# alibaba/pairec

Hardware: AMD Instinct MI355X
Metric: ranked items/sec, 5k-cand DNN rank (recall top-5000 of 100M x 128 -> DNN3 -> fuse -> sort) (higher is better)
Workload: dtype bf16x3; 1 GPU; configs[1]+[2]: recall 5k of 100000000x128 fp32 table in HBM -> 3-layer DNN rank (256-512-256-1, bf16 MFMA with split hi + lo operands = bf16x3, fp32-accurate scores) -> RankScore fusion (fp64) -> ItemRankScore sort; candidates_per_request=5000, table_rows=100000000, dim=128, table_dist=uniform, batches_in_flight=2, contexts=2, all_batches_on_predicted_thresholds=True, batches_re_run_after_a_failed_plan=0, parallelism=1 GPU

## Files before the change

### pairec_amd/csrc/common.hpp

```cpp
#pragma once
#include <hip/hip_runtime.h>

#include <algorithm>
#include <cstdarg>
#include <cstdint>
#include <cstdio>
#include <cstring>
#include <map>
#include <atomic>
#include <memory>
#include <mutex>
#include <shared_mutex>
#include <string>
#include <vector>

#include "../../include/pairec_gpu.h"

namespace pg {

struct PipeRun;
void set_error(const char* fmt, ...);

#define PG_HIP(expr)                                                                           \
    do {                                                                                       \
// ... 440 lines not shown
int ensure_table_r2(pg_ctx* ctx, const pg_table* tc);
int rescreen16_prep_launch(pg_ctx* ctx, const pg_table* t, const RecallScratch& rs, uint32_t nq);
int rescreen16_launch(pg_ctx* ctx, const pg_table* t, const RecallScratch& rs, uint32_t nq);
int screen4m_launch(pg_ctx* ctx, const pg_table* t, const RecallScratch& rs, uint32_t nq, uint32_t row_begin, uint32_t row_end,
                    uint32_t cap1, bool susp2_clean = false);
int topk_merge_strided_locked(pg_ctx* ctx, const uint64_t* d_rows, const float* d_scores, uint32_t nq, uint32_t nlists,
                              uint32_t per_list, size_t row_ls, size_t row_qs, size_t sc_ls, size_t sc_qs, uint32_t k,
                              uint64_t* d_out_rows, float* d_out_scores, uint32_t* d_out_count);
int topk_merge_locked(pg_ctx* ctx, const uint64_t* d_rows, const float* d_scores, uint32_t nq, uint32_t nlists,
                      uint32_t per_list, int list_major, uint32_t k, uint64_t* d_out_rows, float* d_out_scores,
                      uint32_t* d_out_count);

int rank_dnn3_dev_locked(pg_ctx* ctx, const pg_model* m, const pg_table* t, const float* d_user,
                         const uint32_t* d_cand, const uint32_t* d_off, uint32_t n_req, uint32_t n_items,
                         float* d_out, size_t out_stride = 0);
int fm2t_user_embedding_locked(pg_ctx* ctx, const pg_model* m, const float* d_user, uint32_t n_req, float* d_out);
int rank_fm2t_irows_dev_locked(pg_ctx* ctx, const pg_model* m, const pg_item_rows* ir, const float* d_user, const int32_t* d_ufids,
                               const uint32_t* d_cand, const uint32_t* d_off, uint32_t n_req, uint32_t n_items, float* d_out);
int rank_fm2t_rows_dev_locked(pg_ctx* ctx, const pg_model* m, const pg_features* fs, const int32_t* item_field_cols,
                              const float* d_user, const int32_t* d_ufids, const uint32_t* d_cand, const uint32_t* d_off,
                              uint32_t n_req, uint32_t n_items, float* d_out);
int expr_eval_enqueue_locked(pg_ctx* ctx, const pg_expr* e, const double* d_vars, uint32_t n_items, double* d_out,
                             uint32_t* d_err, uint32_t items_per_flag);
void set_expr_arith_error(const pg_expr* e);
constexpr int kMaxRewrites = 8;
void expr_hold(const pg_expr* e);
void expr_release(const pg_expr* e);
struct ExprHold {
    const pg_expr* e = nullptr;
    ExprHold() = default;
    ExprHold(const ExprHold&) = delete;
    ExprHold& operator=(const ExprHold&) = delete;
    void take(const pg_expr* x) {
        if (e) expr_release(e);
        e = x;
        if (e) expr_hold(e);
    }
    ~ExprHold() { if (e) expr_release(e); }
};
int expr_num_rewrites(const pg_expr* e);
const char* expr_rewrite_source(const pg_expr* e, int r);
int expr_rewrite_num_vars(const pg_expr* e, int r);
const char* expr_rewrite_var_name(const pg_expr* e, int r, int i);
int expr_rewrite_eval_enqueue_locked(pg_ctx* ctx, const pg_expr* e, int r, const double* d_vars, uint32_t n_items, double* d_out,
                                     uint32_t* d_err, uint32_t items_per_flag);
int table_gather_locked(pg_ctx* ctx, const pg_table* t, const uint32_t* d_rows, uint32_t n, float* d_out);
// ... 41 lines not shown
```

### pairec_amd/csrc/expr.hip

```cpp
#include "common.hpp"

#include <cmath>
#include <string>
#include <vector>

namespace pg {

enum OpCode : uint32_t { OP_CONST = 0, OP_VAR, OP_ADD, OP_SUB, OP_MUL, OP_DIV, OP_MOD, OP_POW, OP_FNZ,
                         OP_DIVF,
                         OP_NEG };

struct Instr {
    uint32_t op;
    uint32_t arg;
    double val;
};

constexpr int kMaxStack = 32;
constexpr int kMaxProg = 128;

}

struct pg_expr {
    std::string source;
// ... 243 lines not shown
            }
            if (i & 1) {
                a1 *= x1;
                ae += xe;
            }
            x1 *= x1;
            xe <<= 1;
            if (x1 < 0.5) {
                x1 += x1;
                xe--;
            }
        }
        if (y < 0.0) {
            a1 = 1.0 / a1;
            ae = -ae;
        }
        if (ae > 4096) ae = 4096;
        if (ae < -4096) ae = -4096;
        return ldexp(a1, (int)ae);
    }
    return pow(x, y);
}

__global__ void expr_eval_kernel(ExprDev e, const double* __restrict__ vars, uint32_t n_items,
                                 double* __restrict__ out, uint32_t* __restrict__ err, uint32_t items_per_flag) {
    const uint32_t i = blockIdx.x * blockDim.x + threadIdx.x;
    if (i >= n_items) return;
    double st[kMaxStack];
    int sp = 0;
    bool bad = false;
    for (uint32_t pc = 0; pc < e.n; ++pc) {
        const Instr in = e.prog[pc];
        if (in.op == OP_CONST) {
            st[sp++] = in.val;
        } else if (in.op == OP_VAR) {
            st[sp++] = vars[(size_t)in.arg * n_items + i];
        } else {
            if (in.op == OP_NEG) {
                st[sp - 1] = -st[sp - 1];
                continue;
            }
            const double r = st[--sp];
            const double l = st[--sp];
            double v = 0.0;
            switch (in.op) {
                case OP_DIVF: v = l / r; break;
                case OP_ADD: v = l + r; break;
                case OP_SUB: v = l - r; break;
                case OP_MUL: v = l * r; break;
                case OP_DIV:
                    if (r == 0.0) bad = true; else v = l / r;
                    break;
                case OP_MOD: {
                    const long long li = (l == l && fabs(l) < 9223372036854775808.0) ? (long long)l : (long long)0x8000000000000000ull;
                    const long long ri = (r == r && fabs(r) < 9223372036854775808.0) ? (long long)r : (long long)0x8000000000000000ull;
                    if (ri == 0) bad = true;
                    else if (ri == -1) v = 0.0;
                    else v = (double)(li % ri);
                    break;
                }
                case OP_POW: v = go_pow(l, r); break;
                case OP_FNZ: v = (l != 0.0) ? l : r; break;
            }
            st[sp++] = v;
        }
    }
    out[i] = sp > 0 ? st[sp - 1] : 0.0;
    if (bad) atomicOr(err + (items_per_flag ? i / items_per_flag : 0u), 1u);
}

int expr_eval_enqueue_locked(pg_ctx* ctx, const pg_expr* e, const double* d_vars, uint32_t n_items, double* d_out,
                             uint32_t* d_err, uint32_t items_per_flag) {
    if (e->empty) {
        PG_HIP(hipMemsetAsync(d_out, 0, (size_t)n_items * 8, ctx->stream));
    } else {
        ExprDev dev;
        dev.n = (uint32_t)e->prog.size();
        for (size_t i = 0; i < e->prog.size(); ++i) dev.prog[i] = e->prog[i];
        expr_eval_kernel<<<(n_items + 255) / 256, 256, 0, ctx->stream>>>(dev, d_vars, n_items, d_out, d_err, items_per_flag);
        PG_HIP(hipGetLastError());
    }
    return PG_OK;
}

int expr_num_rewrites(const pg_expr* e) { return e ? (int)e->rewrites.size() : 0; }
const char* expr_rewrite_source(const pg_expr* e, int r) { return e->rewrites[(size_t)r].source.c_str(); }
int expr_rewrite_num_vars(const pg_expr* e, int r) { return (int)e->rewrites[(size_t)r].vars.size(); }
const char* expr_rewrite_var_name(const pg_expr* e, int r, int i) { return e->rewrites[(size_t)r].vars[(size_t)i].c_str(); }
int expr_rewrite_eval_enqueue_locked(pg_ctx* ctx, const pg_expr* e, int r, const double* d_vars, uint32_t n_items, double* d_out,
                                     uint32_t* d_err, uint32_t items_per_flag) {
    const pg_expr::Rewrite& rw = e->rewrites[(size_t)r];
    if (rw.failed || rw.prog.empty()) {
        PG_HIP(hipMemsetAsync(d_out, 0, (size_t)n_items * 8, ctx->stream));
        return PG_OK;
    }
    ExprDev dev;
    dev.n = (uint32_t)rw.prog.size();
    for (size_t i = 0; i < rw.prog.size(); ++i) dev.prog[i] = rw.prog[i];
    expr_eval_kernel<<<(n_items + 255) / 256, 256, 0, ctx->stream>>>(dev, d_vars, n_items, d_out, d_err, items_per_flag);
    PG_HIP(hipGetLastError());
    return PG_OK;
}

void set_expr_arith_error(const pg_expr* e) {
// ... 381 lines not shown
```

### pairec_amd/csrc/misc.hip

```cpp
#include "pipeline.hpp"

#include <algorithm>
#include <cstring>
#include <vector>

namespace pg {

__global__ void rows_to_local_kernel(const uint64_t* __restrict__ rows, uint32_t n, uint64_t off,
                                     uint64_t nrows, uint32_t* __restrict__ local,
                                     uint8_t* __restrict__ owned, uint32_t* __restrict__ uni_off, uint32_t uni_nq, uint32_t uni_k) {
    const uint32_t i = blockIdx.x * blockDim.x + threadIdx.x;
    if (uni_off && i <= uni_nq) uni_off[i] = i * uni_k;
    if (i >= n) return;
    const uint64_t r = rows[i];
    const bool mine = r != ~0ull && r >= off && r - off < nrows;
    local[i] = mine ? (uint32_t)(r - off) : 0u;
    if (owned) owned[i] = mine ? 1 : 0;
}

__global__ void widen_kernel(const float* __restrict__ in, uint32_t n, double* __restrict__ out) {
    const uint32_t i = blockIdx.x * blockDim.x + threadIdx.x;
    if (i < n) out[i] = (double)in[i];
}

typedef uint32_t u32x4 __attribute__((ext_vector_type(4)));
__global__ __launch_bounds__(256) void hbm_probe_kernel(const u32x4* __restrict__ p, uint64_t n16,
                                                        uint32_t* __restrict__ sink) {
    uint32_t acc = 0;
    const uint64_t stride = (uint64_t)gridDim.x * blockDim.x;
    uint64_t i = (uint64_t)blockIdx.x * blockDim.x + threadIdx.x;
    for (; i + 3 * stride < n16; i += 4 * stride) {
        const u32x4 a = __builtin_nontemporal_load(&p[i]);
        const u32x4 b = __builtin_nontemporal_load(&p[i + stride]);
        const u32x4 c = __builtin_nontemporal_load(&p[i + 2 * stride]);
        const u32x4 d = __builtin_nontemporal_load(&p[i + 3 * stride]);
// ... 73 lines not shown
    return PG_OK;
}

size_t page_entry_bytes(int n_algos) { return 20 + 4 * (size_t)n_algos; }

int page_launch(hipStream_t st, const uint32_t* d_order, const uint32_t* d_pick, const uint32_t* d_pick_cnt,
                const uint64_t* d_rows, const float* d_recall, const float* d_rank, size_t rank_stride, int n_algos,
                const double* d_fused, uint32_t nq, uint32_t k, uint32_t top_n, char* d_page) {
    const size_t np = (size_t)nq * top_n;
    if (np == 0) return PG_OK;
    uint64_t* p_rows = (uint64_t*)d_page;
    double* p_fused = (double*)(p_rows + np);
    float* p_recall = (float*)(p_fused + np);
    float* p_rank = p_recall + np;
    page_kernel<<<(uint32_t)((np + 255) / 256), 256, 0, st>>>(d_order, d_pick, d_pick_cnt, d_rows, d_recall, d_rank, rank_stride, n_algos,
                                                             d_fused, nq, k, top_n, p_rows, p_fused, p_recall, p_rank);
    PG_HIP(hipGetLastError());
    return PG_OK;
}

int rows_to_local_locked(pg_ctx* ctx, const pg_table* t, const uint64_t* d_rows, uint32_t n, uint32_t* d_local,
                         uint8_t* d_owned) {
    if (n == 0) return PG_OK;
    rows_to_local_kernel<<<(n + 255) / 256, 256, 0, ctx->stream>>>(d_rows, n, t->row_offset, t->rows, d_local, d_owned, nullptr, 0, 0);
    PG_HIP(hipGetLastError());
    return PG_OK;
}

int rows_to_local_offsets_locked(pg_ctx* ctx, const pg_table* t, const uint64_t* d_rows, uint32_t nq, uint32_t k, uint32_t* d_local,
                                 uint32_t* d_off) {
    const uint32_t n = nq * k;
    if (n <= nq) {
        int rc = uniform_offsets_locked(ctx, nq, k, d_off);
        return rc ? rc : rows_to_local_locked(ctx, t, d_rows, n, d_local, nullptr);
    }
    rows_to_local_kernel<<<(n + 255) / 256, 256, 0, ctx->stream>>>(d_rows, n, t->row_offset, t->rows, d_local, nullptr, d_off, nq, k);
    PG_HIP(hipGetLastError());
    return PG_OK;
}

int uniform_offsets_locked(pg_ctx* ctx, uint32_t nq, uint32_t k, uint32_t* d_off) {
    uniform_offsets_kernel<<<(nq + 256) / 256, 256, 0, ctx->stream>>>(nq, k, d_off);
    PG_HIP(hipGetLastError());
    return PG_OK;
}

}

extern "C" {

int pg_hbm_read_probe(pg_ctx* ctx, const pg_table* t, int reps, double* out_gbps) {
    PG_REQUIRE(ctx && t && out_gbps && reps > 0, "pg_hbm_read_probe: bad argument");
    const void* d_buf = t->d;
    const uint64_t bytes = t->rows * (uint64_t)t->dim * 4;
    PG_REQUIRE(bytes >= (1u << 20), "pg_hbm_read_probe: table smaller than 1 MiB");
    std::lock_guard<std::mutex> g(ctx->mu);
    void* sink;
    int rc;
    if ((rc = pg::scratch_reserve(ctx, 4, 4096, &sink))) return rc;
// ... 37 lines not shown
```

### pairec_amd/csrc/pipeline.hip

```cpp
#include "pipeline.hpp"

#include <algorithm>
#include <chrono>
#include <thread>

namespace pg {

struct VarSrc { int8_t src[32]; };
__global__ void bind_vars_kernel(const float* __restrict__ recall, const double* __restrict__ recall64, const float* __restrict__ rank,
                                 size_t rank_stride, uint32_t n, uint32_t nv, VarSrc vs, double* __restrict__ vars,
                                 uint32_t* __restrict__ err, const double* __restrict__ rw, int zero_err) {
    const uint32_t i = blockIdx.x * blockDim.x + threadIdx.x;
    if (zero_err && i < (uint32_t)kMaxQueries) err[i] = 0;
    if (i >= n) return;
    const double a = recall64 ? recall64[i] : (double)recall[i];
    for (uint32_t v = 0; v < nv; ++v) {
        const int sa = vs.src[v];
        vars[(size_t)v * n + i] = sa >= 0 ? (double)rank[(size_t)sa * rank_stride + i] : (sa == -1 ? a : rw[(size_t)(-2 - sa) * n + i]);
    }
}

__global__ void mask_pads_kernel(const uint64_t* __restrict__ rows, uint32_t n, float* __restrict__ rank, size_t rank_stride,
                                 int n_algos, double* __restrict__ fused, int cand, uint64_t row_off, uint64_t nrows,
                                 const uint32_t* __restrict__ count, uint32_t k) {
// ... 99 lines not shown
    const int n_rw = expr_num_rewrites(c.e);
    for (int r = 0; r < n_rw; ++r) wide = std::max(wide, expr_rewrite_num_vars(c.e, r));
    const size_t b_vars = al((size_t)(wide + n_rw) * n * 8);
    if ((rc = scratch_reserve(ctx, 8, b_local + b_off + b_err + b_vars, &buf))) return rc;
    ps->d_local = (uint32_t*)buf;
    ps->d_off = (uint32_t*)((char*)buf + b_local);
    ps->d_err = (uint32_t*)((char*)buf + b_local + b_off);
    ps->d_vars = (double*)((char*)buf + b_local + b_off + b_err);
    ps->c_rows = nullptr; ps->c_rel = nullptr; ps->c_emb = nullptr; ps->c_bail = nullptr;
    if (c.rerank.kind) {
        const size_t nc = (size_t)nq * c.rerank.candidates;
        const size_t b_rows = al(nc * 8), b_rel = al(nc * 8), b_emb = al(nc * c.t->dim * 4), b_bail = al((size_t)kMaxQueries * 4);
        if ((rc = scratch_reserve(ctx, 10, b_rows + b_rel + b_emb + b_bail, &buf))) return rc;
        ps->c_rows = (uint64_t*)buf;
        ps->c_rel = (double*)((char*)buf + b_rows);
        ps->c_emb = (float*)((char*)buf + b_rows + b_rel);
        ps->c_bail = (uint32_t*)((char*)buf + b_rows + b_rel + b_emb);
    }
    return PG_OK;
}

int fuse_scores_enqueue_locked(pg_ctx* ctx, const pg_expr* e, const int* var_src, int nv, const float* d_recall, const float* d_rank,
                               size_t rank_stride, uint32_t n, uint32_t items_per_flag, double* d_vars, uint32_t* d_err, double* d_fused,
                               const double* d_recall64) {
    hipStream_t st = ctx->stream;
    int rc;
    VarSrc vs;
    const int n_rw = expr_num_rewrites(e);
    int wide = std::max(nv, 1);
    for (int r = 0; r < n_rw; ++r) wide = std::max(wide, expr_rewrite_num_vars(e, r));
    double* const d_rw = d_vars + (size_t)wide * n;
    const uint32_t bind_grid = (std::max(n, (uint32_t)kMaxQueries) + 255) / 256;
    bool zeroed = false;
    for (int r = 0, at = nv; r < n_rw; ++r) {
        const int nvr = expr_rewrite_num_vars(e, r);
        for (int i = 0; i < 32; ++i) vs.src[i] = i < nvr ? (int8_t)var_src[at + i] : (int8_t)-1;
        at += nvr;
        if (nvr > 0 || !zeroed) {
            bind_vars_kernel<<<bind_grid, 256, 0, st>>>(d_recall, d_recall64, d_rank, rank_stride, n, (uint32_t)nvr, vs, d_vars, d_err, nullptr, zeroed ? 0 : 1);
            PG_HIP(hipGetLastError());
            zeroed = true;
        }
        if ((rc = expr_rewrite_eval_enqueue_locked(ctx, e, r, d_vars, n, d_rw + (size_t)r * n, d_err, items_per_flag))) return rc;
    }
    for (int i = 0; i < 32; ++i) vs.src[i] = i < nv ? (int8_t)var_src[i] : (int8_t)-1;
    if (nv > 0) {
        bind_vars_kernel<<<bind_grid, 256, 0, st>>>(d_recall, d_recall64, d_rank, rank_stride, n, (uint32_t)nv, vs, d_vars, d_err, d_rw, zeroed ? 0 : 1);
        PG_HIP(hipGetLastError());
    } else if (!zeroed) {
        PG_HIP(hipMemsetAsync(d_err, 0, (size_t)kMaxQueries * 4, st));
    }
    return expr_eval_enqueue_locked(ctx, e, d_vars, n, d_fused, d_err, items_per_flag);
}

int post_fuse_sort_locked(pg_ctx* ctx, const RecommendCall& c, uint32_t q0, uint32_t nq, const PostScratch& ps) {
    const uint32_t n = nq * c.k;
    const size_t o = (size_t)q0 * c.k;
    hipStream_t st = ctx->stream;
    int rc;
    if ((rc = fuse_scores_enqueue_locked(ctx, c.e, c.var_src, c.nv, c.d_recall ? c.d_recall + o : nullptr, c.d_rank + o, c.rank_stride, n, c.k,
                                         ps.d_vars, ps.d_err, c.d_fused + o, c.d_score64 ? c.d_score64 + o : nullptr)))
        return rc;
    if (c.pads || c.cand) {
        mask_pads_kernel<<<(n + 255) / 256, 256, 0, st>>>(c.d_rows + o, n, c.d_rank + o, c.rank_stride, c.planes(), c.d_fused + o, c.cand ? 1 : 0,
                                                          c.t->row_offset, c.t->rows, c.d_cand_count ? c.d_cand_count + q0 : nullptr, c.k);
        PG_HIP(hipGetLastError());
    }
    return sort_dev_locked(ctx, c.d_fused + o, ps.d_off, nq, n, c.k, 1, c.d_order + o);
}

int rerank_select_locked(pg_ctx* ctx, const RecommendCall& c, uint32_t q0, uint32_t nq, const PostScratch& ps) {
    const uint32_t C = c.rerank.candidates;
    const size_t o = (size_t)q0 * c.k;
    if (c.k < C) {
        set_error("recommend: the DPP stage wants %u candidates, the lists hold k = %u", C, c.k);
        return PG_ERR_UNSUPPORTED;
    }
    int rc;
    if ((rc = sorted_head_launch(ctx->stream, c.d_order + o, c.d_rows + o, c.d_fused + o, nq, c.k, C, ps.c_rows, ps.c_rel))) return rc;
    return dpp_norm_relevance_launch(ctx->stream, ps.c_rel, nq, C, c.rerank.dpp.norm_relevance_score, ps.c_bail);
}
int rerank_run_locked(pg_ctx* ctx, const RecommendCall& c, uint32_t q0, uint32_t nq, const PostScratch& ps) {
    const uint32_t C = c.rerank.candidates;
    int rc;
    if ((rc = dpp_run_locked(ctx, ps.c_emb, nullptr, ps.c_rel, nq, C, c.t->dim, 0, c.rerank.dpp.alpha, c.top_n, c.rerank.dpp.window,
                             c.rerank.dpp.normalize_emb, 1, 1, c.d_pick + (size_t)q0 * c.top_n, c.d_pick_cnt + q0)))
        return rc;
    if (c.rerank.dpp.norm_relevance_score)
        return dpp_bail_fix_launch(ctx->stream, ps.c_bail, nq, C, c.top_n, c.d_pick + (size_t)q0 * c.top_n, c.d_pick_cnt + q0);
    return PG_OK;
}

static int recommend_post_locked(pg_ctx* ctx, const RecommendCall& c, uint32_t q0, uint32_t nq, const PostScratch& ps) {
    const uint32_t n = nq * c.k;
    const size_t o = (size_t)q0 * c.k;
    int rc;
    if ((rc = rows_to_local_offsets_locked(ctx, c.t, c.d_rows + o, nq, c.k, ps.d_local, ps.d_off))) return rc;
    for (int a = 0; a < c.n_algos; ++a) {
        const RankAlgoRef& al = c.algos[a];
        float* out = c.d_rank + (size_t)c.plane0[a] * c.rank_stride + o;
        const float* users = c.d_queries + (size_t)q0 * c.t->dim;
        if ((rc = rank_algo_locked(ctx, al, c.t, users, c.d_ufids ? c.d_ufids + (size_t)q0 * c.ufid_stride : nullptr, ps.d_local, ps.d_off, nq, n,
                                   out, c.rank_stride)))
            return rc;
    }
    if ((rc = post_fuse_sort_locked(ctx, c, q0, nq, ps))) return rc;
    if (c.rerank.kind == 1) {
        if (c.t->rows < c.rerank.candidates) {
            set_error("recommend: the DPP stage wants %u candidates, the table has %llu rows", c.rerank.candidates, (unsigned long long)c.t->rows);
            return PG_ERR_UNSUPPORTED;
        }
        if ((rc = rerank_select_locked(ctx, c, q0, nq, ps))) return rc;
        if ((rc = gather_global_rows_launch(ctx->stream, c.t, ps.c_rows, nq * c.rerank.candidates, ps.c_emb))) return rc;
        if ((rc = rerank_run_locked(ctx, c, q0, nq, ps))) return rc;
    }
    return PG_OK;
}

int rank_algo_locked(pg_ctx* ctx, const RankAlgoRef& al, const pg_table* t, const float* d_user, const int32_t* d_ufids,
                     const uint32_t* d_cand, const uint32_t* d_off, uint32_t n_req, uint32_t n_items, float* d_out, size_t out_stride) {
    if (al.m->kind == PG_MODEL_DNN3) return rank_dnn3_dev_locked(ctx, al.m, t, d_user, d_cand, d_off, n_req, n_items, d_out, out_stride);
    if (al.irows) return rank_fm2t_irows_dev_locked(ctx, al.m, al.irows, d_user, d_ufids, d_cand, d_off, n_req, n_items, d_out);
    return rank_fm2t_rows_dev_locked(ctx, al.m, al.fs, al.item_field_cols, d_user, d_ufids, d_cand, d_off, n_req, n_items, d_out);
}

int recommend_enqueue(pg_ctx* ctx, const RecommendCall& c, PipeRun* r, bool first) {
    if (c.t->d_row_map) {
        set_error("recommend: the table is a filtered view (pg_table_view_create) — views serve the recall calls only");
        return PG_ERR_UNSUPPORTED;
// ... 311 lines not shown
```

### pairec_amd/csrc/pipeline.hpp

```cpp
#pragma once
#include "common.hpp"

namespace pg {

struct RecommendCall;
struct PipeRun {
    RecallJob job;
    uint32_t* h_status = nullptr;
    std::vector<hipEvent_t> events;
    hipEvent_t done = nullptr;
    bool patched = false;
};
constexpr uint32_t kExprFlagAt = 320;
constexpr uint32_t kPipeStatusWords = 640;

int pipe_run_acquire(pg_ctx* ctx, PipeRun** out);
void pipe_run_release(pg_ctx* ctx, PipeRun* r);

constexpr int kMaxAlgos = 4;
struct RankAlgoRef {
    const pg_model* m = nullptr;
    const pg_features* fs = nullptr;
    int32_t item_field_cols[16] = {0};
    const pg_item_rows* irows = nullptr;
// ... 31 lines not shown
    int n_planes = 0;
    int planes() const { return n_planes ? n_planes : n_algos; }
    double* d_fused = nullptr;
    uint32_t* d_order = nullptr;
    uint32_t* d_count = nullptr;
    bool pads = false;
    RerankStage rerank;
    uint32_t top_n = 0;
    uint32_t* d_pick = nullptr;
    uint32_t* d_pick_cnt = nullptr;
};
int recommend_bind_vars(const pg_expr* e, const char* const* names, int n_algos, std::vector<int>* var_src, const char* who);
int recommend_enqueue(pg_ctx* ctx, const RecommendCall& c, PipeRun* r, bool first);
int recommend_verify(pg_ctx* ctx, PipeRun* r, bool* ok, const RecommendCall* c = nullptr);
struct PostScratch {
    uint32_t *d_local, *d_off, *d_err;
    double* d_vars;
    uint64_t* c_rows;
    double* c_rel;
    float* c_emb;
    uint32_t* c_bail;
};
int post_scratch(pg_ctx* ctx, const RecommendCall& c, uint32_t nq, PostScratch* ps);
int post_fuse_sort_locked(pg_ctx* ctx, const RecommendCall& c, uint32_t q0, uint32_t nq, const PostScratch& ps);
int fuse_scores_enqueue_locked(pg_ctx* ctx, const pg_expr* e, const int* var_src, int nv, const float* d_recall, const float* d_rank,
                               size_t rank_stride, uint32_t n, uint32_t items_per_flag, double* d_vars, uint32_t* d_err, double* d_fused,
                               const double* d_recall64 = nullptr);
int candidates_trim_locked(pg_ctx* ctx, const pg_trim_rule* rules, uint32_t n_rules, uint32_t nq, uint32_t cap, uint32_t out_cap,
                           const uint64_t* d_rows, const double* d_score, const uint8_t* d_source, const uint32_t* d_count,
                           const double* d_planes_f64, uint32_t n_f64, const uint32_t* d_source_mask, const float* d_planes_f32, uint32_t n_f32,
                           const uint32_t* d_order, uint64_t* d_out_rows, double* d_out_score, uint8_t* d_out_source, double* d_out_planes_f64,
                           uint32_t* d_out_source_mask, float* d_out_planes_f32, uint32_t* d_out_count);
int rerank_select_locked(pg_ctx* ctx, const RecommendCall& c, uint32_t q0, uint32_t nq, const PostScratch& ps);
int rerank_run_locked(pg_ctx* ctx, const RecommendCall& c, uint32_t q0, uint32_t nq, const PostScratch& ps);

int rows_to_local_locked(pg_ctx* ctx, const pg_table* t, const uint64_t* d_rows, uint32_t n, uint32_t* d_local,
                         uint8_t* d_owned);
int uniform_offsets_locked(pg_ctx* ctx, uint32_t nq, uint32_t k, uint32_t* d_off);
int rows_to_local_offsets_locked(pg_ctx* ctx, const pg_table* t, const uint64_t* d_rows, uint32_t nq, uint32_t k, uint32_t* d_local,
                                 uint32_t* d_off);
int sorted_head_launch(hipStream_t st, const uint32_t* d_order, const uint64_t* d_rows, const double* d_fused, uint32_t nq,
                       uint32_t k, uint32_t C, uint64_t* d_c_rows, double* d_c_rel);
int gather_global_rows_launch(hipStream_t st, const pg_table* t, const uint64_t* d_global_rows, uint32_t n, float* d_out);
size_t page_entry_bytes(int n_algos);
int page_launch(hipStream_t st, const uint32_t* d_order, const uint32_t* d_pick, const uint32_t* d_pick_cnt,
                const uint64_t* d_rows, const float* d_recall, const float* d_rank, size_t rank_stride, int n_algos,
                const double* d_fused, uint32_t nq, uint32_t k, uint32_t top_n, char* d_page);
int dpp_norm_relevance_launch(hipStream_t st, double* d_rel, uint32_t nq, uint32_t n, int mode, uint32_t* d_bail);
int dpp_bail_fix_launch(hipStream_t st, const uint32_t* d_bail, uint32_t nq, uint32_t n, uint32_t top_n, uint32_t* d_pick,
                        uint32_t* d_pick_cnt);
bool dpp_norm_relevance_host(const double* rel, uint32_t n, int mode, double* out);
int ssd_run_locked(pg_ctx* ctx, const pg_table* t, const uint32_t* d_cand, const double* d_rel, uint32_t R, uint32_t n,
                   double gamma, uint32_t T, uint32_t window, int normalize_emb, int ensure_pos_similarity, int use_ssd_star,
                   uint32_t* d_out);
bool ssd_batchable(uint32_t d1, uint32_t window);
bool ssd_norm_quality_host(const double* rel, uint32_t n, int mode, double* out);

}
```

### pairec_amd/csrc/rank_mlp.hip

```cpp
#include "rank_mlp.hpp"

#include <algorithm>
#include <cmath>

namespace pg {

template <int PREC, int MB, int NB, int K, bool TR, typename FragOff>
__device__ __forceinline__ void gemm_tile(f32x16 (&acc)[MB][NB], const char* tile, int mrow0,
                                          const char* wpk, FragOff frag, int lane, int tile_lo = 0,
                                          const char* wpk_lo = nullptr) {
    constexpr int ES = PREC ? 2 : 4;
    constexpr int ROWB = K * ES;
    constexpr int SW = (ROWB / 16 < 16 ? ROWB / 16 : 16) - 1;
    const int i32 = lane & 31, h = lane >> 5;
    if constexpr (PREC == 2) {
        static_assert(TR, "split bf16: transposed accumulators only");
#pragma unroll
        for (int ks = 0; ks < K / 16; ++ks) {
            bf16x8 bh[NB], bl[NB];
#pragma unroll
            for (int nb = 0; nb < NB; ++nb) {
                bh[nb] = *reinterpret_cast<const bf16x8*>(wpk + frag(nb, ks) + lane * 16);
                bl[nb] = *reinterpret_cast<const bf16x8*>(wpk_lo + frag(nb, ks) + lane * 16);
            }
// ... 568 lines not shown
    build_tiles_wide_body(blockIdx.x, req_offsets, n_req, tile_req, tile_item0, tile_cnt, n_tiles, req_tile0, tile_items);
}
struct TileTableArgs {
    const uint32_t* req_offsets;
    uint32_t n_req;
    uint32_t *tile_req, *tile_item0, *tile_cnt, *n_tiles, *req_tile0;
    uint32_t tile_items;
    uint32_t blocks;
};

static int build_tiles_launch(pg_ctx* ctx, const uint32_t* d_off, uint32_t n_req, uint32_t max_tiles, uint32_t tile_items,
                              uint32_t* tile_req, uint32_t* tile_item0, uint32_t* tile_cnt, uint32_t* n_tiles,
                              uint32_t* req_tile0) {
    if (n_req <= kTilesLdsReqs)
        build_tiles_wide_kernel<<<(max_tiles + 255) / 256, 256, 0, ctx->stream>>>(d_off, n_req, tile_req, tile_item0, tile_cnt,
                                                                                  n_tiles, req_tile0, tile_items);
    else
        build_tiles_kernel<<<1, 1024, 0, ctx->stream>>>(d_off, n_req, tile_req, tile_item0, tile_cnt, n_tiles, req_tile0,
                                                        tile_items);
    PG_HIP(hipGetLastError());
    return PG_OK;
}

__global__ void dnn3_user_partial_kernel(const float* __restrict__ user, uint32_t du,
                                         const float* __restrict__ w1u, const float* __restrict__ b1,
                                         uint32_t h1, int prec, float* __restrict__ c1) {
    const uint32_t r = blockIdx.x;
    const uint32_t j = blockIdx.y * blockDim.x + threadIdx.x;
    if (j >= h1) return;
    const float* const u = user + (size_t)r * du;
    float acc = b1[j];
    uint32_t k = 0;
    for (; k + 64 <= du; k += 64) {
        float wv[64];
#pragma unroll
        for (int i = 0; i < 64; ++i) wv[i] = w1u[(size_t)(k + i) * h1 + j];
#pragma unroll
        for (int i = 0; i < 64; ++i) acc = __fmaf_rn(round_prec(u[k + i], prec), wv[i], acc);
    }
    for (; k + 8 <= du; k += 8) {
        float wv[8], uv[8];
#pragma unroll
        for (int i = 0; i < 8; ++i) {
            wv[i] = w1u[(size_t)(k + i) * h1 + j];
            uv[i] = round_prec(u[k + i], prec);
        }
#pragma unroll
        for (int i = 0; i < 8; ++i) acc = __fmaf_rn(uv[i], wv[i], acc);
    }
    for (; k < du; ++k) acc = __fmaf_rn(round_prec(u[k], prec), w1u[(size_t)k * h1 + j], acc);
    c1[(size_t)r * h1 + j] = acc;
}

__device__ __forceinline__ void fm2t_user_prefix(uint32_t r, uint32_t tid, const float* const* __restrict__ field_emb,
                                                 const float* const* __restrict__ field_lin,
                                                 const int32_t* __restrict__ user_field_ids, uint32_t vocab, float fm_b,
                                                 float* __restrict__ fm_user, uint32_t nuf, uint32_t fk) {
    if (!user_field_ids) return;
    if (tid < fk) {
        float s = 0.0f, q = 0.0f;
        for (uint32_t f = 0; f < nuf; ++f) {
            int32_t id = user_field_ids[(size_t)r * nuf + f];
            id = id < 0 ? 0 : (id >= (int32_t)vocab ? (int32_t)vocab - 1 : id);
            const float v = field_emb[f][(size_t)id * fk + tid];
            s = s + v;
            q = __fmaf_rn(v, v, q);
        }
        fm_user[(size_t)r * kFmUserStride + 1 + tid] = s;
        fm_user[(size_t)r * kFmUserStride + 1 + kFmMaxK + tid] = q;
    }
    if (tid == 64) {
        float lin = fm_b;
        for (uint32_t f = 0; f < nuf; ++f) {
            int32_t id = user_field_ids[(size_t)r * nuf + f];
// ... 362 lines not shown
    return PG_ERR_UNSUPPORTED;
}

int rank_dnn3_dev_locked(pg_ctx* ctx, const pg_model* m, const pg_table* t,
                                const float* d_user, const uint32_t* d_cand, const uint32_t* d_off,
                                uint32_t n_req, uint32_t n_items, float* d_out, size_t out_stride) {
    if (n_items == 0 || n_req == 0) return PG_OK;
    const uint32_t max_tiles = n_items / 32 + n_req;
    RankScratch rs;
    int rc;
    if ((rc = rank_scratch(ctx, n_req, max_tiles, m->h1, &rs))) return rc;
    const bool no_ws = ctx->knobs.rank_no_ws;
    const bool ws = m->prec == 1 && !no_ws && m->h1 == 512 && m->h2 == 256 && t->dim == 128;
    const bool rs_k = m->prec == 1 && !no_ws && t->dim == 128 && dnn3_rs_shape(m->h1, m->h2);
    const bool ls_k = m->prec == 1 && !no_ws && t->dim == 128 && dnn3_ls_shape(m->h1, m->h2);
    const bool x3_k = m->prec == 2 && !no_ws && t->dim == 128 && dnn3_x3_shape(m->h1, m->h2);
    const bool h2_k = m->f16_nprod && x3_k;
    if (m->f16_nprod) {
        m->f16_calls++;
        if (!h2_k) m->f16_calls_whole++;
    }
    const uint32_t grid128 = n_items / kBM + n_req;
    if (!ctx->timers_off) PG_HIP(hipEventRecord(ctx->ev[2], ctx->stream));
    if ((rc = build_tiles_launch(ctx, d_off, n_req, max_tiles, ws || rs_k ? (uint32_t)kWsItems : (uint32_t)kBM, rs.tile_req, rs.tile_item0,
                                 rs.tile_cnt, rs.n_tiles, rs.req_tile0)))
        return rc;
    dnn3_user_partial_kernel<<<dim3(n_req, (m->h1 + 255) / 256), 256, 0, ctx->stream>>>(
        d_user, m->d_user, m->w1u, m->b1, m->h1, m->prec, rs.c1);
    MlpArgs a{};
    a.tile_req = rs.tile_req;
    a.tile_item0 = rs.tile_item0;
    a.tile_cnt = rs.tile_cnt;
    a.n_tiles = rs.n_tiles;
    a.tab = t->d;
    a.tab_rows = (uint32_t)t->rows;
    a.tab_dim = t->dim;
    a.cand_rows = d_cand;
    a.c1 = rs.c1;
    a.c1_stride = m->h1;
    a.w3 = m->w3;
    a.w3_stride = 0;
    a.b3 = m->b3;
    a.b2 = m->b2;
    a.w1p = m->w1p;
    a.w2p = m->w2p;
    a.w1p_lo = m->w1p_lo;
    a.w2p_lo = m->w2p_lo;
    a.out = d_out;
    a.n_out = m->n_out;
    a.out_stride = out_stride ? out_stride : (size_t)n_items;
    a.b3v = m->b3v;
// ... 681 lines not shown
```

### pairec_amd/csrc/recall.hip

```cpp
#include "common.hpp"
#include "bitonic_reg.hpp"
#include "split_sort.hpp"

#include <type_traits>

namespace pg {

typedef float f32x16 __attribute__((ext_vector_type(16)));
typedef float f32x4 __attribute__((ext_vector_type(4)));

constexpr int kPieceRows = 32;
constexpr int kPieceCols = 32;
constexpr int kPieceBytes = kPieceRows * kPieceCols * 4;
constexpr int kPieceDmas = kPieceBytes / 1024;
constexpr int kPieceQuads = kPieceCols / 4;
constexpr int kRingSlots = 4;
constexpr int kScanWaves = 8;
constexpr int kScanLdsRing = kScanWaves * kRingSlots * kPieceBytes;
constexpr int kStageCap = 280;
constexpr int kStageBytes = kStageCap * 12 + 512;
constexpr int kScanLds = kScanLdsRing + kScanWaves * kStageBytes;

__device__ __forceinline__ uint32_t f32_ordered_bits(float f) {
    const uint32_t b = __float_as_uint(f);
// ... 1627 lines not shown
    const float* S = pred + 128;
    float sq = 0.0f;
    for (int i = 0; i < 128; ++i) sq = __fmaf_rn(S[i * 128 + t], qs[i], sq);
    double v = (double)sq * (double)qs[t], m = (double)pred[t] * (double)qs[t];
    for (int off = 32; off > 0; off >>= 1) {
        v += __shfl_xor(v, off, 64);
        m += __shfl_xor(m, off, 64);
    }
    if ((t & 63) == 0) { red[t >> 6][0] = v; red[t >> 6][1] = m; }
    __syncthreads();
    if (t == 0) {
        const double var = red[0][0] + red[1][0], mean = red[0][1] + red[1][1];
        const float m = (float)mean, sg = var > 0.0 ? (float)sqrt(var) : 0.0f;
        ms[2 * q] = m;
        ms[2 * q + 1] = sg;
        if (thr) {
            float t = __fmaf_rn(z_lo, sg, m);
            t = t - fabsf(t) * 1e-6f;
            if (!(sg > 0.0f) || !(t == t) || fabsf(t) > 1e30f) t = __builtin_inff();
            thr[q] = t;
        }
    }
}
__global__ void pred_update_kernel(const float* __restrict__ thr, const float* __restrict__ ms, const uint32_t* __restrict__ cnt,
                                   uint32_t nq, uint32_t k, double* __restrict__ stats) {
    const uint32_t q = threadIdx.x;
    double z = 0.0, z2 = 0.0, n = 0.0, mn = 1e300;
    if (q < nq && cnt[q] >= k && ms[2 * q + 1] > 0.0f) {
        const float t = thr[q];
        if (t == t && fabsf(t) < 1e30f) {
            z = ((double)t - (double)ms[2 * q]) / (double)ms[2 * q + 1];
            z2 = z * z;
            n = 1.0;
            mn = z;
        }
    }
    for (int off = 32; off > 0; off >>= 1) {
        z += __shfl_xor(z, off, 64);
        z2 += __shfl_xor(z2, off, 64);
        n += __shfl_xor(n, off, 64);
        const double o = __shfl_xor(mn, off, 64);
        mn = o < mn ? o : mn;
    }
    if ((q & 63) == 0 && n > 0.0) {
        atomicAdd(&stats[4], n);
        atomicAdd(&stats[0], n);
        atomicAdd(&stats[1], z);
        atomicAdd(&stats[2], z2);
// ... 247 lines not shown
    PG_HIP(hipMemsetAsync(t->dnorm2, 0, n_blk * sizeof(float), ctx->stream));
    PG_HIP(hipMemsetAsync(d_max, 0, 8, ctx->stream));
    if (t->dim == 64) table_shadow_kernel<64><<<grid, 256, 0, ctx->stream>>>(t->d, t->rows, t->d16, d_max, d_bad, t->dnorm2);
    else table_shadow_kernel<128><<<grid, 256, 0, ctx->stream>>>(t->d, t->rows, t->d16, d_max, d_bad, t->dnorm2);
    PG_HIP(hipGetLastError());
    PG_HIP(hipMemcpyAsync(ctx->h_status + 300, d_max, 8, hipMemcpyDeviceToHost, ctx->stream));
    PG_HIP(hipStreamSynchronize(ctx->stream));
    float mx;
    memcpy(&mx, ctx->h_status + 300, 4);
    t->all_finite = ctx->h_status[301] == 0;
    t->max_norm = sqrtf(mx) * 1.0001f;
    t->shadow_is_i8 = false;
    t->stats_valid = true;
    return PG_OK;
}

constexpr uint32_t kPredStatsAt = 260;
constexpr uint32_t kI4mStatAt = 272;
constexpr uint32_t kStatusCopyWords = kI4mStatAt + 5;
static_assert(kStatusCopyWords <= 300 && kStatusCopyWords <= kRecallStatusWords, "the status block ends in front of the words other calls keep in ctx->h_status");
static_assert(kIndexStatAt > kMaxQueries && kIndexStatAt + 12 <= kStatusCopyWords, "an index plan's status words");

__global__ void status_pack_kernel(const uint32_t* __restrict__ overflow, uint32_t nq, uint32_t rec_ovf_word,
                                   const uint32_t* __restrict__ pred_stats, const uint32_t* __restrict__ pairs_word,
                                   const uint32_t* __restrict__ susp, const uint32_t* __restrict__ rescored,
                                   const uint32_t* __restrict__ cand_seen, uint32_t* __restrict__ out) {
    const uint32_t t = threadIdx.x;
    uint32_t v1 = (susp && t < nq) ? susp[t] : 0u, v3 = (rescored && t < nq) ? rescored[t] : 0u, v4 = (cand_seen && t < nq) ? cand_seen[t] : 0u;
#pragma unroll
    for (int off = 32; off > 0; off >>= 1) {
        v1 += __shfl_xor(v1, off, 64);
        v3 += __shfl_xor(v3, off, 64);
        v4 += __shfl_xor(v4, off, 64);
    }
    __shared__ uint32_t s[3][4];
    if ((t & 63) == 0) { s[0][t >> 6] = v1; s[1][t >> 6] = v3; s[2][t >> 6] = v4; }
    out[1 + t] = t < nq ? overflow[1 + t] : 0u;
    if (t < 10) out[kPredStatsAt + t] = pred_stats ? pred_stats[t] : 0u;
    __syncthreads();
    if (t == 0) {
        out[0] = overflow[0];
        out[kI4mStatAt] = pairs_word ? *pairs_word : 0u;
        out[kI4mStatAt + 1] = s[0][0] + s[0][1] + s[0][2] + s[0][3];
        out[kI4mStatAt + 2] = overflow[rec_ovf_word];
        out[kI4mStatAt + 3] = s[1][0] + s[1][1] + s[1][2] + s[1][3];
        out[kI4mStatAt + 4] = s[2][0] + s[2][1] + s[2][2] + s[2][3];
    }
}

static int ensure_pred_model(pg_ctx* ctx, const pg_table* tc) {
    pg_table* t = const_cast<pg_table*>(tc);
    std::lock_guard<std::mutex> build_guard(g_stats_build_mu);
    if (t->pred_model) return PG_OK;
    const size_t bytes = (size_t)(128 + 128 * 128) * 4 + 5 * 8;
    if (!t->d_pred && hipMalloc((void**)&t->d_pred, bytes) != hipSuccess) {
        (void)hipGetLastError();
        t->d_pred = nullptr;
        return PG_OK;
    }
    PG_HIP(hipMemsetAsync(t->d_pred, 0, bytes, ctx->stream));
    const uint64_t n_sample = t->rows < (1u << 20) ? t->rows : (1u << 20);
// ... 697 lines not shown
    } else {
        r.exact_chunks = plan == kSafe && j->filter.col;
        const double growth = kn.chunk_growth > 1.0 ? kn.chunk_growth : (j->screen && !r.exact_chunks ? 2.0 : 4.0);
        if ((rc = r.grow_scan(j->nblocks, 1, j->k, growth, plan == kSafe))) return rc;
    }
    if (j->timers) PG_HIP(hipEventRecord((*j->events)[1], ctx->stream));
    if ((rc = final_launch(ctx, rs.cand[r.cur], rs.cnt, rs.cap, j->nq, j->k, t->row_offset, j->d_out_rows,
                           j->d_out_scores, j->d_count)))
        return rc;
    if (t->d_row_map) {
        const uint64_t n = (uint64_t)j->nq * j->k;
        compact_map_rows_kernel<<<(uint32_t)((n + 255) / 256), 256, 0, ctx->stream>>>(j->d_out_rows, n, t->d_row_map, t->map_offset, t->rows);
        PG_HIP(hipGetLastError());
    }
    if (j->l2) {
        const uint64_t n = (uint64_t)j->nq * j->k;
        negate_kernel<<<(uint32_t)((n + 255) / 256), 256, 0, ctx->stream>>>(j->d_out_scores, n);
        PG_HIP(hipGetLastError());
    }
    if (refined) {
        refine_verify_kernel<<<1, kMaxQueries, 0, ctx->stream>>>(rs.thr, rs.thr_ref, j->d_count, j->nq);
        PG_HIP(hipGetLastError());
    }
    if (observe) {
        double* stats = reinterpret_cast<double*>(t->d_pred + 128 + 128 * 128);
        pred_update_kernel<<<1, kMaxQueries, 0, ctx->stream>>>(rs.thr, rs.pred_ms, j->d_count, j->nq, j->k < j->rows ? j->k : j->rows, stats);
        PG_HIP(hipGetLastError());
    }
    j->susp_stat = j->screen && (plan == kPilot || plan == kPredict) && r.last_full_screened;
    j->stat_wide = j->susp_stat && !r.last_was_i4m;
    {
        const uint32_t* const susp = j->susp_stat ? (r.last_was_i4m ? rs.susp2_cnt : rs.susp_cnt) : nullptr;
        status_pack_kernel<<<1, kMaxQueries, 0, ctx->stream>>>(
            rs.overflow, j->nq, kRecOvfWord, observe ? reinterpret_cast<const uint32_t*>(t->d_pred + 128 + 128 * 128) : nullptr,
            j->susp_stat && r.last_was_i4m ? rs.susp2_cnt + kI4mMaxQueries : nullptr, susp, j->susp_stat && r.last_was_r2 ? rs.susp2w_cnt : susp,
            j->susp_stat ? rs.cnt_seen : nullptr, rs.status);
        PG_HIP(hipGetLastError());
    }
    if (j->d_out_count)
        PG_HIP(hipMemcpyAsync(j->d_out_count, j->d_count, 4 * j->nq, hipMemcpyDeviceToDevice, ctx->stream));
    PG_HIP(hipMemcpyAsync(j->h_status, rs.status, 4 * (size_t)kStatusCopyWords, hipMemcpyDeviceToHost, ctx->stream));
    j->n_ev = r.n_ev;
    j->refined = refined;
    j->enqueued_plan = plan;
    j->observed = observe;
    j->next_plan++;
    return PG_OK;
}

int recall_job_check(RecallJob* j, bool* ok_out) {
    pg_ctx* ctx = j->ctx;
    const int plan = j->enqueued_plan;
    float ms = 0.f;
    if (j->timers) PG_HIP(hipEventElapsedTime(&ms, (*j->events)[0], (*j->events)[1]));
    j->total_ms += ms;
    for (uint32_t i = 1; j->timers && i < j->n_ev; ++i) {
        PG_HIP(hipEventElapsedTime(&ms, (*j->events)[2 * i], (*j->events)[2 * i + 1]));
// ... 702 lines not shown
```

Measured before the change: 275.5 million ranked items/s.

## Fold small pipeline kernels and memsets into neighbouring launches

Several tiny launches are merged into adjacent kernels. The fusion expression with no rewrites now reads recall and rank planes directly instead of going through a bind kernel and vars buffer. The error-flag memset moves into rows_to_local, the tile-table build is folded into the DNN user-partial kernel as an extra grid row, and the pred_update kernel is merged into status_pack. The goal is to cut per-launch overhead on a latency-bound 5k-candidate pipeline. The cost is more complex kernels and ordering assumptions, for example that the extra tile-building blocks are guaranteed to finish before later kernels read the tile table.

```diff
diff --git a/pairec_amd/csrc/common.hpp b/pairec_amd/csrc/common.hpp
--- a/pairec_amd/csrc/common.hpp
+++ b/pairec_amd/csrc/common.hpp
@@ -486,6 +486,9 @@
                               uint32_t n_req, uint32_t n_items, float* d_out);
 int expr_eval_enqueue_locked(pg_ctx* ctx, const pg_expr* e, const double* d_vars, uint32_t n_items, double* d_out,
                              uint32_t* d_err, uint32_t items_per_flag);
+int expr_eval_planes_enqueue_locked(pg_ctx* ctx, const pg_expr* e, const int* var_src, int nv, const float* d_recall,
+                                    const double* d_recall64, const float* d_rank, size_t rank_stride, uint32_t n_items,
+                                    double* d_out, uint32_t* d_err, uint32_t items_per_flag);
 void set_expr_arith_error(const pg_expr* e);
 constexpr int kMaxRewrites = 8;
 void expr_hold(const pg_expr* e);
diff --git a/pairec_amd/csrc/expr.hip b/pairec_amd/csrc/expr.hip
--- a/pairec_amd/csrc/expr.hip
+++ b/pairec_amd/csrc/expr.hip
@@ -289,10 +289,9 @@
     return pow(x, y);
 }
 
-__global__ void expr_eval_kernel(ExprDev e, const double* __restrict__ vars, uint32_t n_items,
-                                 double* __restrict__ out, uint32_t* __restrict__ err, uint32_t items_per_flag) {
-    const uint32_t i = blockIdx.x * blockDim.x + threadIdx.x;
-    if (i >= n_items) return;
+template <class Var>
+__device__ __forceinline__ void expr_eval_item(const ExprDev& e, uint32_t i, Var var, double* __restrict__ out,
+                                               uint32_t* __restrict__ err, uint32_t items_per_flag) {
     double st[kMaxStack];
     int sp = 0;
     bool bad = false;
@@ -301,7 +300,7 @@
         if (in.op == OP_CONST) {
             st[sp++] = in.val;
         } else if (in.op == OP_VAR) {
-            st[sp++] = vars[(size_t)in.arg * n_items + i];
+            st[sp++] = var(in.arg);
         } else {
             if (in.op == OP_NEG) {
                 st[sp - 1] = -st[sp - 1];
@@ -336,6 +335,25 @@
     if (bad) atomicOr(err + (items_per_flag ? i / items_per_flag : 0u), 1u);
 }
 
+__global__ void expr_eval_kernel(ExprDev e, const double* __restrict__ vars, uint32_t n_items,
+                                 double* __restrict__ out, uint32_t* __restrict__ err, uint32_t items_per_flag) {
+    const uint32_t i = blockIdx.x * blockDim.x + threadIdx.x;
+    if (i >= n_items) return;
+    expr_eval_item(e, i, [&](uint32_t v) { return vars[(size_t)v * n_items + i]; }, out, err, items_per_flag);
+}
+
+struct ExprVarSrc { int8_t src[32]; };
+__global__ void expr_eval_planes_kernel(ExprDev e, ExprVarSrc vs, const float* __restrict__ recall, const double* __restrict__ recall64,
+                                        const float* __restrict__ rank, size_t rank_stride, uint32_t n_items,
+                                        double* __restrict__ out, uint32_t* __restrict__ err, uint32_t items_per_flag) {
+    const uint32_t i = blockIdx.x * blockDim.x + threadIdx.x;
+    if (i >= n_items) return;
+    expr_eval_item(e, i, [&](uint32_t v) {
+        const int sa = vs.src[v & 31u];
+        return sa >= 0 ? (double)rank[(size_t)sa * rank_stride + i] : (recall64 ? recall64[i] : (double)recall[i]);
+    }, out, err, items_per_flag);
+}
+
 int expr_eval_enqueue_locked(pg_ctx* ctx, const pg_expr* e, const double* d_vars, uint32_t n_items, double* d_out,
                              uint32_t* d_err, uint32_t items_per_flag) {
     if (e->empty) {
@@ -347,6 +365,21 @@
         expr_eval_kernel<<<(n_items + 255) / 256, 256, 0, ctx->stream>>>(dev, d_vars, n_items, d_out, d_err, items_per_flag);
         PG_HIP(hipGetLastError());
     }
+    return PG_OK;
+}
+
+int expr_eval_planes_enqueue_locked(pg_ctx* ctx, const pg_expr* e, const int* var_src, int nv, const float* d_recall,
+                                    const double* d_recall64, const float* d_rank, size_t rank_stride, uint32_t n_items,
+                                    double* d_out, uint32_t* d_err, uint32_t items_per_flag) {
+    if (e->empty) return expr_eval_enqueue_locked(ctx, e, nullptr, n_items, d_out, d_err, items_per_flag);
+    ExprDev dev;
+    dev.n = (uint32_t)e->prog.size();
+    for (size_t i = 0; i < e->prog.size(); ++i) dev.prog[i] = e->prog[i];
+    ExprVarSrc vs;
+    for (int i = 0; i < 32; ++i) vs.src[i] = i < nv ? (int8_t)var_src[i] : (int8_t)-1;
+    expr_eval_planes_kernel<<<(n_items + 255) / 256, 256, 0, ctx->stream>>>(dev, vs, d_recall, d_recall64, d_rank, rank_stride, n_items,
+                                                                            d_out, d_err, items_per_flag);
+    PG_HIP(hipGetLastError());
     return PG_OK;
 }
 
diff --git a/pairec_amd/csrc/misc.hip b/pairec_amd/csrc/misc.hip
--- a/pairec_amd/csrc/misc.hip
+++ b/pairec_amd/csrc/misc.hip
@@ -8,9 +8,11 @@
 
 __global__ void rows_to_local_kernel(const uint64_t* __restrict__ rows, uint32_t n, uint64_t off,
                                      uint64_t nrows, uint32_t* __restrict__ local,
-                                     uint8_t* __restrict__ owned, uint32_t* __restrict__ uni_off, uint32_t uni_nq, uint32_t uni_k) {
+                                     uint8_t* __restrict__ owned, uint32_t* __restrict__ uni_off, uint32_t uni_nq, uint32_t uni_k,
+                                     uint32_t* __restrict__ zero) {
     const uint32_t i = blockIdx.x * blockDim.x + threadIdx.x;
     if (uni_off && i <= uni_nq) uni_off[i] = i * uni_k;
+    if (zero && i < (uint32_t)kMaxQueries) zero[i] = 0;
     if (i >= n) return;
     const uint64_t r = rows[i];
     const bool mine = r != ~0ull && r >= off && r - off < nrows;
@@ -130,19 +132,20 @@
 int rows_to_local_locked(pg_ctx* ctx, const pg_table* t, const uint64_t* d_rows, uint32_t n, uint32_t* d_local,
                          uint8_t* d_owned) {
     if (n == 0) return PG_OK;
-    rows_to_local_kernel<<<(n + 255) / 256, 256, 0, ctx->stream>>>(d_rows, n, t->row_offset, t->rows, d_local, d_owned, nullptr, 0, 0);
+    rows_to_local_kernel<<<(n + 255) / 256, 256, 0, ctx->stream>>>(d_rows, n, t->row_offset, t->rows, d_local, d_owned, nullptr, 0, 0, nullptr);
     PG_HIP(hipGetLastError());
     return PG_OK;
 }
 
 int rows_to_local_offsets_locked(pg_ctx* ctx, const pg_table* t, const uint64_t* d_rows, uint32_t nq, uint32_t k, uint32_t* d_local,
-                                 uint32_t* d_off) {
+                                 uint32_t* d_off, uint32_t* d_zero) {
     const uint32_t n = nq * k;
     if (n <= nq) {
+        if (d_zero) PG_HIP(hipMemsetAsync(d_zero, 0, (size_t)kMaxQueries * 4, ctx->stream));
         int rc = uniform_offsets_locked(ctx, nq, k, d_off);
         return rc ? rc : rows_to_local_locked(ctx, t, d_rows, n, d_local, nullptr);
     }
-    rows_to_local_kernel<<<(n + 255) / 256, 256, 0, ctx->stream>>>(d_rows, n, t->row_offset, t->rows, d_local, nullptr, d_off, nq, k);
+    rows_to_local_kernel<<<(n + 255) / 256, 256, 0, ctx->stream>>>(d_rows, n, t->row_offset, t->rows, d_local, nullptr, d_off, nq, k, d_zero);
     PG_HIP(hipGetLastError());
     return PG_OK;
 }
diff --git a/pairec_amd/csrc/pipeline.hip b/pairec_amd/csrc/pipeline.hip
--- a/pairec_amd/csrc/pipeline.hip
+++ b/pairec_amd/csrc/pipeline.hip
@@ -145,16 +145,20 @@
 
 int fuse_scores_enqueue_locked(pg_ctx* ctx, const pg_expr* e, const int* var_src, int nv, const float* d_recall, const float* d_rank,
                                size_t rank_stride, uint32_t n, uint32_t items_per_flag, double* d_vars, uint32_t* d_err, double* d_fused,
-                               const double* d_recall64) {
+                               const double* d_recall64, bool err_zeroed) {
     hipStream_t st = ctx->stream;
     int rc;
     VarSrc vs;
     const int n_rw = expr_num_rewrites(e);
+    if (n_rw == 0) {
+        if (!err_zeroed) PG_HIP(hipMemsetAsync(d_err, 0, (size_t)kMaxQueries * 4, st));
+        return expr_eval_planes_enqueue_locked(ctx, e, var_src, nv, d_recall, d_recall64, d_rank, rank_stride, n, d_fused, d_err, items_per_flag);
+    }
     int wide = std::max(nv, 1);
     for (int r = 0; r < n_rw; ++r) wide = std::max(wide, expr_rewrite_num_vars(e, r));
     double* const d_rw = d_vars + (size_t)wide * n;
     const uint32_t bind_grid = (std::max(n, (uint32_t)kMaxQueries) + 255) / 256;
-    bool zeroed = false;
+    bool zeroed = err_zeroed;
     for (int r = 0, at = nv; r < n_rw; ++r) {
         const int nvr = expr_rewrite_num_vars(e, r);
         for (int i = 0; i < 32; ++i) vs.src[i] = i < nvr ? (int8_t)var_src[at + i] : (int8_t)-1;
@@ -176,13 +180,13 @@
     return expr_eval_enqueue_locked(ctx, e, d_vars, n, d_fused, d_err, items_per_flag);
 }
 
-int post_fuse_sort_locked(pg_ctx* ctx, const RecommendCall& c, uint32_t q0, uint32_t nq, const PostScratch& ps) {
+int post_fuse_sort_locked(pg_ctx* ctx, const RecommendCall& c, uint32_t q0, uint32_t nq, const PostScratch& ps, bool err_zeroed) {
     const uint32_t n = nq * c.k;
     const size_t o = (size_t)q0 * c.k;
     hipStream_t st = ctx->stream;
     int rc;
     if ((rc = fuse_scores_enqueue_locked(ctx, c.e, c.var_src, c.nv, c.d_recall ? c.d_recall + o : nullptr, c.d_rank + o, c.rank_stride, n, c.k,
-                                         ps.d_vars, ps.d_err, c.d_fused + o, c.d_score64 ? c.d_score64 + o : nullptr)))
+                                         ps.d_vars, ps.d_err, c.d_fused + o, c.d_score64 ? c.d_score64 + o : nullptr, err_zeroed)))
         return rc;
     if (c.pads || c.cand) {
         mask_pads_kernel<<<(n + 255) / 256, 256, 0, st>>>(c.d_rows + o, n, c.d_rank + o, c.rank_stride, c.planes(), c.d_fused + o, c.cand ? 1 : 0,
@@ -218,7 +222,7 @@
     const uint32_t n = nq * c.k;
     const size_t o = (size_t)q0 * c.k;
     int rc;
-    if ((rc = rows_to_local_offsets_locked(ctx, c.t, c.d_rows + o, nq, c.k, ps.d_local, ps.d_off))) return rc;
+    if ((rc = rows_to_local_offsets_locked(ctx, c.t, c.d_rows + o, nq, c.k, ps.d_local, ps.d_off, ps.d_err))) return rc;
     for (int a = 0; a < c.n_algos; ++a) {
         const RankAlgoRef& al = c.algos[a];
         float* out = c.d_rank + (size_t)c.plane0[a] * c.rank_stride + o;
@@ -227,7 +231,7 @@
                                    out, c.rank_stride)))
             return rc;
     }
-    if ((rc = post_fuse_sort_locked(ctx, c, q0, nq, ps))) return rc;
+    if ((rc = post_fuse_sort_locked(ctx, c, q0, nq, ps, true))) return rc;
     if (c.rerank.kind == 1) {
         if (c.t->rows < c.rerank.candidates) {
             set_error("recommend: the DPP stage wants %u candidates, the table has %llu rows", c.rerank.candidates, (unsigned long long)c.t->rows);
diff --git a/pairec_amd/csrc/pipeline.hpp b/pairec_amd/csrc/pipeline.hpp
--- a/pairec_amd/csrc/pipeline.hpp
+++ b/pairec_amd/csrc/pipeline.hpp
@@ -77,10 +77,10 @@
     uint32_t* c_bail;
 };
 int post_scratch(pg_ctx* ctx, const RecommendCall& c, uint32_t nq, PostScratch* ps);
-int post_fuse_sort_locked(pg_ctx* ctx, const RecommendCall& c, uint32_t q0, uint32_t nq, const PostScratch& ps);
+int post_fuse_sort_locked(pg_ctx* ctx, const RecommendCall& c, uint32_t q0, uint32_t nq, const PostScratch& ps, bool err_zeroed = false);
 int fuse_scores_enqueue_locked(pg_ctx* ctx, const pg_expr* e, const int* var_src, int nv, const float* d_recall, const float* d_rank,
                                size_t rank_stride, uint32_t n, uint32_t items_per_flag, double* d_vars, uint32_t* d_err, double* d_fused,
-                               const double* d_recall64 = nullptr);
+                               const double* d_recall64 = nullptr, bool err_zeroed = false);
 int candidates_trim_locked(pg_ctx* ctx, const pg_trim_rule* rules, uint32_t n_rules, uint32_t nq, uint32_t cap, uint32_t out_cap,
                            const uint64_t* d_rows, const double* d_score, const uint8_t* d_source, const uint32_t* d_count,
                            const double* d_planes_f64, uint32_t n_f64, const uint32_t* d_source_mask, const float* d_planes_f32, uint32_t n_f32,
@@ -93,7 +93,7 @@
                          uint8_t* d_owned);
 int uniform_offsets_locked(pg_ctx* ctx, uint32_t nq, uint32_t k, uint32_t* d_off);
 int rows_to_local_offsets_locked(pg_ctx* ctx, const pg_table* t, const uint64_t* d_rows, uint32_t nq, uint32_t k, uint32_t* d_local,
-                                 uint32_t* d_off);
+                                 uint32_t* d_off, uint32_t* d_zero = nullptr);
 int sorted_head_launch(hipStream_t st, const uint32_t* d_order, const uint64_t* d_rows, const double* d_fused, uint32_t nq,
                        uint32_t k, uint32_t C, uint64_t* d_c_rows, double* d_c_rel);
 int gather_global_rows_launch(hipStream_t st, const pg_table* t, const uint64_t* d_global_rows, uint32_t n, float* d_out);
diff --git a/pairec_amd/csrc/rank_mlp.hip b/pairec_amd/csrc/rank_mlp.hip
--- a/pairec_amd/csrc/rank_mlp.hip
+++ b/pairec_amd/csrc/rank_mlp.hip
@@ -614,11 +614,9 @@
     return PG_OK;
 }
 
-__global__ void dnn3_user_partial_kernel(const float* __restrict__ user, uint32_t du,
-                                         const float* __restrict__ w1u, const float* __restrict__ b1,
-                                         uint32_t h1, int prec, float* __restrict__ c1) {
-    const uint32_t r = blockIdx.x;
-    const uint32_t j = blockIdx.y * blockDim.x + threadIdx.x;
+__device__ __forceinline__ void dnn3_user_partial_body(uint32_t r, uint32_t j, const float* __restrict__ user, uint32_t du,
+                                                       const float* __restrict__ w1u, const float* __restrict__ b1,
+                                                       uint32_t h1, int prec, float* __restrict__ c1) {
     if (j >= h1) return;
     const float* const u = user + (size_t)r * du;
     float acc = b1[j];
@@ -642,6 +640,19 @@
     }
     for (; k < du; ++k) acc = __fmaf_rn(round_prec(u[k], prec), w1u[(size_t)k * h1 + j], acc);
     c1[(size_t)r * h1 + j] = acc;
+}
+__global__ __launch_bounds__(256) void dnn3_user_partial_kernel(const float* __restrict__ user, uint32_t du,
+                                                                const float* __restrict__ w1u, const float* __restrict__ b1,
+                                                                uint32_t h1, int prec, float* __restrict__ c1, uint32_t n_req,
+                                                                TileTableArgs tt) {
+    if (tt.blocks && blockIdx.y + 1 == gridDim.y) {
+        if (blockIdx.x < tt.blocks)
+            build_tiles_wide_body(blockIdx.x, tt.req_offsets, tt.n_req, tt.tile_req, tt.tile_item0, tt.tile_cnt, tt.n_tiles, tt.req_tile0,
+                                  tt.tile_items);
+        return;
+    }
+    if (blockIdx.x >= n_req) return;
+    dnn3_user_partial_body(blockIdx.x, blockIdx.y * blockDim.x + threadIdx.x, user, du, w1u, b1, h1, prec, c1);
 }
 
 __device__ __forceinline__ void fm2t_user_prefix(uint32_t r, uint32_t tid, const float* const* __restrict__ field_emb,
@@ -1050,11 +1061,15 @@
     }
     const uint32_t grid128 = n_items / kBM + n_req;
     if (!ctx->timers_off) PG_HIP(hipEventRecord(ctx->ev[2], ctx->stream));
-    if ((rc = build_tiles_launch(ctx, d_off, n_req, max_tiles, ws || rs_k ? (uint32_t)kWsItems : (uint32_t)kBM, rs.tile_req, rs.tile_item0,
-                                 rs.tile_cnt, rs.n_tiles, rs.req_tile0)))
+    const uint32_t tile_items = ws || rs_k ? (uint32_t)kWsItems : (uint32_t)kBM;
+    TileTableArgs tt{};
+    if (n_req <= kTilesLdsReqs)
+        tt = TileTableArgs{d_off, n_req, rs.tile_req, rs.tile_item0, rs.tile_cnt, rs.n_tiles, rs.req_tile0, tile_items, (max_tiles + 255) / 256};
+    else if ((rc = build_tiles_launch(ctx, d_off, n_req, max_tiles, tile_items, rs.tile_req, rs.tile_item0, rs.tile_cnt, rs.n_tiles, rs.req_tile0)))
         return rc;
-    dnn3_user_partial_kernel<<<dim3(n_req, (m->h1 + 255) / 256), 256, 0, ctx->stream>>>(
-        d_user, m->d_user, m->w1u, m->b1, m->h1, m->prec, rs.c1);
+    const uint32_t yb = (m->h1 + 255) / 256;
+    dnn3_user_partial_kernel<<<dim3(std::max(n_req, tt.blocks), tt.blocks ? yb + 1 : yb), 256, 0, ctx->stream>>>(
+        d_user, m->d_user, m->w1u, m->b1, m->h1, m->prec, rs.c1, n_req, tt);
     MlpArgs a{};
     a.tile_req = rs.tile_req;
     a.tile_item0 = rs.tile_item0;
diff --git a/pairec_amd/csrc/recall.hip b/pairec_amd/csrc/recall.hip
--- a/pairec_amd/csrc/recall.hip
+++ b/pairec_amd/csrc/recall.hip
@@ -1673,8 +1673,8 @@
         }
     }
 }
-__global__ void pred_update_kernel(const float* __restrict__ thr, const float* __restrict__ ms, const uint32_t* __restrict__ cnt,
-                                   uint32_t nq, uint32_t k, double* __restrict__ stats) {
+__device__ __forceinline__ void pred_update_body(const float* __restrict__ thr, const float* __restrict__ ms, const uint32_t* __restrict__ cnt,
+                                                 uint32_t nq, uint32_t k, double* stats) {
     const uint32_t q = threadIdx.x;
     double z = 0.0, z2 = 0.0, n = 0.0, mn = 1e300;
     if (q < nq && cnt[q] >= k && ms[2 * q + 1] > 0.0f) {
@@ -1968,10 +1968,16 @@
 static_assert(kIndexStatAt > kMaxQueries && kIndexStatAt + 12 <= kStatusCopyWords, "an index plan's status words");
 
 __global__ void status_pack_kernel(const uint32_t* __restrict__ overflow, uint32_t nq, uint32_t rec_ovf_word,
-                                   const uint32_t* __restrict__ pred_stats, const uint32_t* __restrict__ pairs_word,
+                                   double* pred_stats, const float* __restrict__ pred_thr, const float* __restrict__ pred_ms,
+                                   const uint32_t* __restrict__ pred_cnt, uint32_t pred_k, const uint32_t* __restrict__ pairs_word,
                                    const uint32_t* __restrict__ susp, const uint32_t* __restrict__ rescored,
                                    const uint32_t* __restrict__ cand_seen, uint32_t* __restrict__ out) {
     const uint32_t t = threadIdx.x;
+    if (pred_stats) {
+        pred_update_body(pred_thr, pred_ms, pred_cnt, nq, pred_k, pred_stats);
+        __threadfence();
+        __syncthreads();
+    }
     uint32_t v1 = (susp && t < nq) ? susp[t] : 0u, v3 = (rescored && t < nq) ? rescored[t] : 0u, v4 = (cand_seen && t < nq) ? cand_seen[t] : 0u;
 #pragma unroll
     for (int off = 32; off > 0; off >>= 1) {
@@ -1982,7 +1988,9 @@
     __shared__ uint32_t s[3][4];
     if ((t & 63) == 0) { s[0][t >> 6] = v1; s[1][t >> 6] = v3; s[2][t >> 6] = v4; }
     out[1 + t] = t < nq ? overflow[1 + t] : 0u;
-    if (t < 10) out[kPredStatsAt + t] = pred_stats ? pred_stats[t] : 0u;
+    if (t < 10)
+        out[kPredStatsAt + t] =
+            pred_stats ? __hip_atomic_load(reinterpret_cast<const uint32_t*>(pred_stats) + t, __ATOMIC_RELAXED, __HIP_MEMORY_SCOPE_AGENT) : 0u;
     __syncthreads();
     if (t == 0) {
         out[0] = overflow[0];
@@ -2726,17 +2734,13 @@
         refine_verify_kernel<<<1, kMaxQueries, 0, ctx->stream>>>(rs.thr, rs.thr_ref, j->d_count, j->nq);
         PG_HIP(hipGetLastError());
     }
-    if (observe) {
-        double* stats = reinterpret_cast<double*>(t->d_pred + 128 + 128 * 128);
-        pred_update_kernel<<<1, kMaxQueries, 0, ctx->stream>>>(rs.thr, rs.pred_ms, j->d_count, j->nq, j->k < j->rows ? j->k : j->rows, stats);
-        PG_HIP(hipGetLastError());
-    }
     j->susp_stat = j->screen && (plan == kPilot || plan == kPredict) && r.last_full_screened;
     j->stat_wide = j->susp_stat && !r.last_was_i4m;
     {
         const uint32_t* const susp = j->susp_stat ? (r.last_was_i4m ? rs.susp2_cnt : rs.susp_cnt) : nullptr;
         status_pack_kernel<<<1, kMaxQueries, 0, ctx->stream>>>(
-            rs.overflow, j->nq, kRecOvfWord, observe ? reinterpret_cast<const uint32_t*>(t->d_pred + 128 + 128 * 128) : nullptr,
+            rs.overflow, j->nq, kRecOvfWord, observe ? reinterpret_cast<double*>(t->d_pred + 128 + 128 * 128) : nullptr, rs.thr, rs.pred_ms,
+            j->d_count, j->k < j->rows ? j->k : j->rows,
             j->susp_stat && r.last_was_i4m ? rs.susp2_cnt + kI4mMaxQueries : nullptr, susp, j->susp_stat && r.last_was_r2 ? rs.susp2w_cnt : susp,
             j->susp_stat ? rs.cnt_seen : nullptr, rs.status);
         PG_HIP(hipGetLastError());
```

Result: no change. 275.0 million ranked items/s (-0.2%).
